# rampasek/GraphGPS

Hardware: NVIDIA H100
Metric: graphs/sec GPSLayer fwd+bwd (higher is better)
Workload: dtype f32

## Files before the change

### graphgps_b200/csrc/attention.cu

```cuda
#include "kernels.cuh"

namespace gps {

namespace {

constexpr int kWarpsPerBlock = 4;

__device__ __forceinline__ int find_graph(const int* __restrict__ gptr, int B, int node) {
  int lo = 0, hi = B;
  while (hi - lo > 1) {
    int mid = (lo + hi) >> 1;
    if (gptr[mid] <= node) lo = mid; else hi = mid;
  }
  return lo;
}

template <int LPR>
__device__ __forceinline__ float group_sum(float v) {
#pragma unroll
  for (int o = LPR / 2; o > 0; o >>= 1) v += __shfl_xor_sync(0xffffffffu, v, o);
  return v;
}

__device__ __forceinline__ int warp_max_i(int v) {
#pragma unroll
  for (int o = 16; o > 0; o >>= 1) v = max(v, __shfl_xor_sync(0xffffffffu, v, o));
  return v;
}

struct DropQuad {
  Philox4 r;
  uint32_t thr;
  float keep_scale;
};
__device__ __forceinline__ void drop_quad_refresh(DropQuad& q, float p, uint64_t seed, uint64_t offset, int head, int i, int jl) {
  q.r = philox4x32(seed, offset + (uint64_t)(GPS_SITE_ATTN_P + head), ((uint64_t)i << 20) | (uint64_t)(jl >> 2));
}
__device__ __forceinline__ float drop_quad_scale(const DropQuad& q, int jl) {
  const int k = jl & 3;
  const uint32_t bits = k == 0 ? q.r.v[0] : k == 1 ? q.r.v[1] : k == 2 ? q.r.v[2] : q.r.v[3];
  return bits >= q.thr ? q.keep_scale : 0.f;
}
__device__ __forceinline__ void drop_quad_init(DropQuad& q, float p) {
  q.thr = (uint32_t)fminf(p * 4294967296.f, 4294967295.f);
  q.keep_scale = 1.f / (1.f - p);
}

template <int VW> struct VecT;
template <> struct VecT<4> { using T = float4; };
template <> struct VecT<1> { using T = float; };

template <int VW> __device__ __forceinline__ typename VecT<VW>::T vld(const float* p);
template <> __device__ __forceinline__ float4 vld<4>(const float* p) { return ld4(p); }
template <> __device__ __forceinline__ float vld<1>(const float* p) { return *p; }
template <int VW> __device__ __forceinline__ typename VecT<VW>::T vzero();
template <> __device__ __forceinline__ float4 vzero<4>() { return f4zero(); }
template <> __device__ __forceinline__ float vzero<1>() { return 0.f; }
__device__ __forceinline__ void vst(float* p, float4 v) { st4(p, v); }
__device__ __forceinline__ void vst(float* p, float v) { *p = v; }
__device__ __forceinline__ float4 vscale(float4 a, float s) { return f4scale(a, s); }
__device__ __forceinline__ float vscale(float a, float s) { return a * s; }
__device__ __forceinline__ float vdot(float4 a, float4 b) { return a.x * b.x + a.y * b.y + a.z * b.z + a.w * b.w; }
__device__ __forceinline__ float vdot(float a, float b) { return a * b; }
__device__ __forceinline__ void vplanes_store(const Planes& p, int64_t r, int64_t c, float4 v) { planes_store4(p, r, c, v); }
__device__ __forceinline__ void vplanes_store(const Planes& p, int64_t r, int64_t c, float v) {
  const __nv_bfloat16 h = __float2bfloat16_rn(v);
  p.hi[r * p.ld + c] = h;
  if (p.lo) p.lo[r * p.ld + c] = __float2bfloat16_rn(v - __bfloat162float(h));
}

template <int CH, int LPR, int VW>
__device__ __forceinline__ void load_slice(typename VecT<VW>::T* dst, const float* row, int sub, int nch, bool ok) {
#pragma unroll
  for (int c = 0; c < CH; ++c) {
    int ch = sub + c * LPR;
    dst[c] = (ok && ch < nch) ? vld<VW>(row + ch * VW) : vzero<VW>();
  }
}
template <int CH, int LPR, int VW>
__device__ __forceinline__ void store_slice(const typename VecT<VW>::T* src, float* row, int sub, int nch) {
#pragma unroll
  for (int c = 0; c < CH; ++c) {
    int ch = sub + c * LPR;
    if (ch < nch) vst(row + ch * VW, src[c]);
  }
}
template <int CH, int LPR, int VW>
__device__ __forceinline__ void store_slice_planes(const typename VecT<VW>::T* src, const Planes& p, int64_t r, int64_t col0,
                                                   int sub, int nch) {
  if (!p.hi) return;
#pragma unroll
  for (int c = 0; c < CH; ++c) {
    int ch = sub + c * LPR;
    if (ch < nch) vplanes_store(p, r, col0 + ch * VW, src[c]);
  }
}
template <int CH, typename V>
__device__ __forceinline__ float dot_slice(const V* a, const V* b) {
  float s = 0.f;
#pragma unroll
  for (int c = 0; c < CH; ++c) s += vdot(a[c], b[c]);
  return s;
}

struct AttnArgs {
  const int* gptr; int B; int N; int H; int hd;
  const float* Q; const float* K; const float* V; int64_t ld;
  float* O; const float* Oc; const float* dO; int64_t ldo;
  float* lse; const float* lsec; float* delta; const float* deltac;
  float* dQ; float* dK; float* dV; int64_t ldg;
  float scale; float p_drop; uint64_t seed, offset;
  const unsigned long long* offset_dev;
  Planes Op, dQp, dKp, dVp;
  int smem_rows;
  const float* bias; int64_t nmax; float* gbias;
};
__device__ __forceinline__ uint64_t eff_offset(const AttnArgs& a) {
  return a.offset + ((a.p_drop > 0.f && a.offset_dev) ? *a.offset_dev : 0ull);
}

struct StagedRows {
  const float* x; int64_t ldx;
  const float* y; int64_t ldy;
};
template <int RPB, int VW>
__device__ __forceinline__ StagedRows stage_rows(const AttnArgs& a, const float* X, int64_t ldX, const float* Y, int64_t ldY,
                                                 int h, float* sm) {
  const int64_t hoff = (int64_t)h * a.hd;
  StagedRows r{X + hoff, ldX, Y + hoff, ldY};
  const int r0 = blockIdx.x * RPB;
  if (a.smem_rows <= 0 || r0 >= a.N) return r;
  const int last = min(r0 + RPB, a.N) - 1;
  const int kmin = a.gptr[find_graph(a.gptr, a.B, r0)];
  const int R = a.gptr[find_graph(a.gptr, a.B, last) + 1] - kmin;
  if (R > a.smem_rows) return r;
  const int pitch = a.hd + 4, nch = VW == 4 ? a.hd >> 2 : a.hd;
  float* sx = sm;
  float* sy = sm + (int64_t)a.smem_rows * pitch;
  for (int idx = threadIdx.x; idx < R * nch; idx += blockDim.x) {
    const int row = idx / nch, c = idx - row * nch;
    vst(sx + row * pitch + c * VW, vld<VW>(X + (int64_t)(kmin + row) * ldX + hoff + c * VW));
    vst(sy + row * pitch + c * VW, vld<VW>(Y + (int64_t)(kmin + row) * ldY + hoff + c * VW));
  }
  __syncthreads();
  r.x = sx - (int64_t)kmin * pitch; r.ldx = pitch;
  r.y = sy - (int64_t)kmin * pitch; r.ldy = pitch;
  return r;
}

template <int CH, int LPR, bool BIAS, int VW>
__global__ void __launch_bounds__(kWarpsPerBlock * 32) k_attn_fwd(AttnArgs a) {
  extern __shared__ float attn_sm[];
  using V = typename VecT<VW>::T;
  constexpr int RPW = 32 / LPR;
  const int warp = threadIdx.x >> 5, lane = threadIdx.x & 31;
  const int sub = lane % LPR, rloc = lane / LPR;
  const int h = blockIdx.y;
  const int i = (blockIdx.x * kWarpsPerBlock + warp) * RPW + rloc;
  const bool row_ok = i < a.N;
  const int nch = a.hd / VW;
  const uint64_t offs = eff_offset(a);
  int gs = 0, n = 0;
  const float* brow = nullptr;
  if (row_ok) {
    int g = find_graph(a.gptr, a.B, i);
    gs = a.gptr[g];
    n = a.gptr[g + 1] - gs;
    if constexpr (BIAS) brow = a.bias + (((int64_t)g * a.H + h) * a.nmax + (i - gs)) * a.nmax;
  }
  const int nloop = warp_max_i(n);
  const int64_t hoff = (int64_t)h * a.hd;
  V q[CH], o[CH];
  load_slice<CH, LPR, VW>(q, a.Q + (int64_t)(row_ok ? i : 0) * a.ld + hoff, sub, nch, row_ok);
#pragma unroll
  for (int c = 0; c < CH; ++c) {
    q[c] = vscale(q[c], a.scale);
    o[c] = vzero<VW>();
  }
  float m = -INFINITY, l = 0.f;
  const bool use_drop = a.p_drop > 0.f;
  DropQuad dq;
  drop_quad_init(dq, a.p_drop);
  const StagedRows kv = stage_rows<RPW * kWarpsPerBlock, VW>(a, a.K, a.ld, a.V, a.ld, h, attn_sm);
  V kc[CH], vc[CH];
  load_slice<CH, LPR, VW>(kc, kv.x + (int64_t)gs * kv.ldx, sub, nch, n > 0);
  load_slice<CH, LPR, VW>(vc, kv.y + (int64_t)gs * kv.ldy, sub, nch, n > 0);
  float bc = 0.f;
  if constexpr (BIAS) bc = n > 0 ? brow[0] : 0.f;
  for (int jl = 0; jl < nloop; ++jl) {
    if (use_drop && (jl & 3) == 0) drop_quad_refresh(dq, a.p_drop, a.seed, offs, h, i, jl);
    const bool valid = jl < n;
    const bool nvalid = jl + 1 < n;
    const int jn = gs + (nvalid ? jl + 1 : 0);
    V kn[CH], vn[CH];
    load_slice<CH, LPR, VW>(kn, kv.x + (int64_t)jn * kv.ldx, sub, nch, nvalid);
    load_slice<CH, LPR, VW>(vn, kv.y + (int64_t)jn * kv.ldy, sub, nch, nvalid);
    float bn = 0.f;
    if constexpr (BIAS) bn = nvalid ? brow[jl + 1] : 0.f;
    float s = group_sum<LPR>(dot_slice<CH>(q, kc));
    if constexpr (BIAS) s += bc;
    s = valid ? s : -INFINITY;
    const float m_new = fmaxf(m, s);
    const float corr = (m_new == -INFINITY) ? 1.f : __expf(m - m_new);
    const float p = valid ? __expf(s - m_new) : 0.f;
    l = l * corr + p;
    const float pd = use_drop ? p * drop_quad_scale(dq, jl) : p;
#pragma unroll
    for (int c = 0; c < CH; ++c) {
      if constexpr (VW == 4) {
        o[c].x = o[c].x * corr + pd * vc[c].x;
        o[c].y = o[c].y * corr + pd * vc[c].y;
        o[c].z = o[c].z * corr + pd * vc[c].z;
        o[c].w = o[c].w * corr + pd * vc[c].w;
      } else {
        o[c] = o[c] * corr + pd * vc[c];
      }
      kc[c] = kn[c];
      vc[c] = vn[c];
    }
    if constexpr (BIAS) bc = bn;
    m = m_new;
  }
  if (row_ok) {
    const float inv = 1.f / l;
#pragma unroll
    for (int c = 0; c < CH; ++c) o[c] = vscale(o[c], inv);
    store_slice<CH, LPR, VW>(o, a.O + (int64_t)i * a.ldo + hoff, sub, nch);
    store_slice_planes<CH, LPR, VW>(o, a.Op, i, hoff, sub, nch);
    if (sub == 0) a.lse[(int64_t)i * a.H + h] = m + __logf(l);
  }
}

template <int VW>
__global__ void k_attn_delta(AttnArgs a) {
  using V = typename VecT<VW>::T;
  const int64_t t = ((int64_t)blockIdx.x * blockDim.x + threadIdx.x) >> 3;
  const int sub = threadIdx.x & 7;
  const bool ok = t < (int64_t)a.N * a.H;
  const int64_t i = ok ? t / a.H : 0;
  const int h = ok ? (int)(t - i * a.H) : 0;
  const V* go = reinterpret_cast<const V*>(a.dO + i * a.ldo + (int64_t)h * a.hd);
  const V* oo = reinterpret_cast<const V*>(a.Oc + i * a.ldo + (int64_t)h * a.hd);
  float acc = 0.f;
  if (ok)
    for (int c = sub; c < a.hd / VW; c += 8) {
      const V x = __ldg(go + c), y = __ldg(oo + c);
      acc += vdot(x, y);
    }
  acc += __shfl_xor_sync(0xffffffffu, acc, 4);
  acc += __shfl_xor_sync(0xffffffffu, acc, 2);
  acc += __shfl_xor_sync(0xffffffffu, acc, 1);
  if (ok && sub == 0) a.delta[t] = acc;
}

template <int CH, int LPR, bool BIAS, int VW>
__device__ __forceinline__ void attn_bwd_q_body(const AttnArgs& a, float* attn_sm) {
  using V = typename VecT<VW>::T;
  constexpr int RPW = 32 / LPR;
  const int warp = threadIdx.x >> 5, lane = threadIdx.x & 31;
  const int sub = lane % LPR, rloc = lane / LPR;
  const int h = blockIdx.y;
  const int i = (blockIdx.x * kWarpsPerBlock + warp) * RPW + rloc;
  const bool row_ok = i < a.N;
  const int nch = a.hd / VW;
  const uint64_t offs = eff_offset(a);
  int gs = 0, n = 0;
  int64_t brow = 0;
  if (row_ok) {
    int g = find_graph(a.gptr, a.B, i);
    gs = a.gptr[g];
    n = a.gptr[g + 1] - gs;
    if constexpr (BIAS) brow = (((int64_t)g * a.H + h) * a.nmax + (i - gs)) * a.nmax;
  }
  const int nloop = warp_max_i(n);
  const int64_t hoff = (int64_t)h * a.hd;
  const int ir = row_ok ? i : 0;
  V q[CH], go[CH], gq[CH];
  load_slice<CH, LPR, VW>(q, a.Q + (int64_t)ir * a.ld + hoff, sub, nch, row_ok);
  load_slice<CH, LPR, VW>(go, a.dO + (int64_t)ir * a.ldo + hoff, sub, nch, row_ok);
  {
    const float dl = row_ok ? a.deltac[(int64_t)i * a.H + h] : 0.f;
#pragma unroll
    for (int c = 0; c < CH; ++c) gq[c] = vzero<VW>();
    const float lse = row_ok ? a.lsec[(int64_t)i * a.H + h] : 0.f;
#pragma unroll
    for (int c = 0; c < CH; ++c) q[c] = vscale(q[c], a.scale);
    const bool use_drop = a.p_drop > 0.f;
    DropQuad dq;
    drop_quad_init(dq, a.p_drop);
    const StagedRows kv = stage_rows<RPW * kWarpsPerBlock, VW>(a, a.K, a.ld, a.V, a.ld, h, attn_sm);
    V kk[CH], vv[CH];
    load_slice<CH, LPR, VW>(kk, kv.x + (int64_t)gs * kv.ldx, sub, nch, n > 0);
    load_slice<CH, LPR, VW>(vv, kv.y + (int64_t)gs * kv.ldy, sub, nch, n > 0);
    float bc = 0.f;
    if constexpr (BIAS) bc = n > 0 ? a.bias[brow] : 0.f;
    for (int jl = 0; jl < nloop; ++jl) {
      if (use_drop && (jl & 3) == 0) drop_quad_refresh(dq, a.p_drop, a.seed, offs, h, i, jl);
      const bool valid = jl < n;
      const bool nvalid = jl + 1 < n;
      const int jn = gs + (nvalid ? jl + 1 : 0);
      V kn[CH], vn[CH];
      load_slice<CH, LPR, VW>(kn, kv.x + (int64_t)jn * kv.ldx, sub, nch, nvalid);
      load_slice<CH, LPR, VW>(vn, kv.y + (int64_t)jn * kv.ldy, sub, nch, nvalid);
      float bn = 0.f;
      if constexpr (BIAS) bn = nvalid ? a.bias[brow + jl + 1] : 0.f;
      float s = dot_slice<CH>(q, kk), dp = dot_slice<CH>(go, vv);
#pragma unroll
      for (int ofs = LPR / 2; ofs > 0; ofs >>= 1) {
        s += __shfl_xor_sync(0xffffffffu, s, ofs);
        dp += __shfl_xor_sync(0xffffffffu, dp, ofs);
      }
      if constexpr (BIAS) s += bc;
      const float p = valid ? __expf(s - lse) : 0.f;
      const float ds = p * (dp * (use_drop ? drop_quad_scale(dq, jl) : 1.f) - dl);
      if constexpr (BIAS) {
        if (a.gbias && valid && sub == 0) a.gbias[brow + jl] = ds;
        bc = bn;
      }
#pragma unroll
      for (int c = 0; c < CH; ++c) {
        if constexpr (VW == 4) {
          gq[c].x += ds * kk[c].x;
          gq[c].y += ds * kk[c].y;
          gq[c].z += ds * kk[c].z;
          gq[c].w += ds * kk[c].w;
        } else {
          gq[c] += ds * kk[c];
        }
        kk[c] = kn[c];
        vv[c] = vn[c];
      }
    }
  }
  if (row_ok) {
#pragma unroll
    for (int c = 0; c < CH; ++c) gq[c] = vscale(gq[c], a.scale);
    store_slice<CH, LPR, VW>(gq, a.dQ + (int64_t)i * a.ldg + hoff, sub, nch);
    store_slice_planes<CH, LPR, VW>(gq, a.dQp, i, hoff, sub, nch);
  }
}

template <int CH, int LPR, bool BIAS, int VW>
__device__ __forceinline__ void attn_bwd_kv_body(const AttnArgs& a, float* attn_sm) {
  using V = typename VecT<VW>::T;
  constexpr int RPW = 32 / LPR;
  const int warp = threadIdx.x >> 5, lane = threadIdx.x & 31;
  const int sub = lane % LPR, rloc = lane / LPR;
  const int h = blockIdx.y;
  const int j = (blockIdx.x * kWarpsPerBlock + warp) * RPW + rloc;
  const bool row_ok = j < a.N;
  const int nch = a.hd / VW;
  const uint64_t offs = eff_offset(a);
  int gs = 0, n = 0;
  const float* bcol = nullptr;
  if (row_ok) {
    int g = find_graph(a.gptr, a.B, j);
    gs = a.gptr[g];
    n = a.gptr[g + 1] - gs;
    if constexpr (BIAS) bcol = a.bias + ((int64_t)g * a.H + h) * a.nmax * a.nmax + (j - gs);
  }
  const int nloop = warp_max_i(n);
  const int jl = j - gs;
  const int64_t hoff = (int64_t)h * a.hd;
  const int jr = row_ok ? j : 0;
  V kk[CH], vv[CH], gk[CH], gv[CH];
  load_slice<CH, LPR, VW>(kk, a.K + (int64_t)jr * a.ld + hoff, sub, nch, row_ok);
  load_slice<CH, LPR, VW>(vv, a.V + (int64_t)jr * a.ld + hoff, sub, nch, row_ok);
#pragma unroll
  for (int c = 0; c < CH; ++c) {
    gk[c] = vzero<VW>();
    gv[c] = vzero<VW>();
  }
  const StagedRows qd = stage_rows<RPW * kWarpsPerBlock, VW>(a, a.Q, a.ld, a.dO, a.ldo, h, attn_sm);
  V q[CH], go[CH];
  load_slice<CH, LPR, VW>(q, qd.x + (int64_t)gs * qd.ldx, sub, nch, n > 0);
  load_slice<CH, LPR, VW>(go, qd.y + (int64_t)gs * qd.ldy, sub, nch, n > 0);
  for (int il = 0; il < nloop; ++il) {
    const bool valid = il < n;
    const int i = gs + (valid ? il : 0);
    const bool nvalid = il + 1 < n;
    const int in_ = gs + (nvalid ? il + 1 : 0);
    V qn[CH], gon[CH];
    load_slice<CH, LPR, VW>(qn, qd.x + (int64_t)in_ * qd.ldx, sub, nch, nvalid);
    load_slice<CH, LPR, VW>(gon, qd.y + (int64_t)in_ * qd.ldy, sub, nch, nvalid);
    float s = dot_slice<CH>(q, kk), dp = dot_slice<CH>(go, vv);
#pragma unroll
    for (int ofs = LPR / 2; ofs > 0; ofs >>= 1) {
      s += __shfl_xor_sync(0xffffffffu, s, ofs);
      dp += __shfl_xor_sync(0xffffffffu, dp, ofs);
    }
    const float lse = valid ? a.lsec[(int64_t)i * a.H + h] : 0.f;
    const float dl = valid ? a.deltac[(int64_t)i * a.H + h] : 0.f;
    float p;
    if constexpr (BIAS) p = valid ? __expf(s * a.scale + bcol[(int64_t)il * a.nmax] - lse) : 0.f;
    else p = valid ? __expf(s * a.scale - lse) : 0.f;
    float dsc = 1.f;
    if (a.p_drop > 0.f) {
      DropQuad dq;
      drop_quad_init(dq, a.p_drop);
      drop_quad_refresh(dq, a.p_drop, a.seed, offs, h, i, jl);
      dsc = drop_quad_scale(dq, jl);
    }
    const float pd = p * dsc;
    const float ds = p * (dp * dsc - dl) * a.scale;
#pragma unroll
    for (int c = 0; c < CH; ++c) {
      if constexpr (VW == 4) {
        gk[c].x += ds * q[c].x; gk[c].y += ds * q[c].y; gk[c].z += ds * q[c].z; gk[c].w += ds * q[c].w;
        gv[c].x += pd * go[c].x; gv[c].y += pd * go[c].y; gv[c].z += pd * go[c].z; gv[c].w += pd * go[c].w;
      } else {
        gk[c] += ds * q[c];
        gv[c] += pd * go[c];
      }
      q[c] = qn[c];
      go[c] = gon[c];
    }
  }
  if (row_ok) {
    store_slice<CH, LPR, VW>(gk, a.dK + (int64_t)j * a.ldg + hoff, sub, nch);
    store_slice<CH, LPR, VW>(gv, a.dV + (int64_t)j * a.ldg + hoff, sub, nch);
    store_slice_planes<CH, LPR, VW>(gk, a.dKp, j, hoff, sub, nch);
    store_slice_planes<CH, LPR, VW>(gv, a.dVp, j, hoff, sub, nch);
  }
}

template <int CH, int LPR, bool BIAS, int VW>
__global__ void __launch_bounds__(kWarpsPerBlock * 32) k_attn_bwd(AttnArgs a) {
  extern __shared__ float attn_sm[];
  if (blockIdx.z == 0) attn_bwd_kv_body<CH, LPR, BIAS, VW>(a, attn_sm);
  else attn_bwd_q_body<CH, LPR, BIAS, VW>(a, attn_sm);
}

enum { KFWD = 0, KBWD = 1 };

constexpr int kStageBytes = 72 * 1024;

static bool attn_vec4(const AttnArgs& a, int which) {
  return a.hd % 4 == 0 && a.ld % 4 == 0 && a.ldo % 4 == 0 && (which == KFWD || a.ldg % 4 == 0);
}

template <int CH, int LPR, bool BIAS, int VW>
static void launch_one(int which, const AttnArgs& a0, cudaStream_t stream) {
  constexpr int RPW = 32 / LPR;
  AttnArgs a = a0;
  static const bool stage_on = [] {
    const char* e = getenv("GPS_B200_ATTN_STAGE");
    return e && e[0] == '1';
  }();
  const int pitch = a.hd + 4;
  a.smem_rows = (stage_on && a.B > 0 && a.N < 64LL * a.B) ? kStageBytes / (2 * pitch * 4) : 0;
  const size_t smem = a.smem_rows > 0 ? (size_t)2 * a.smem_rows * pitch * 4 : 0;
  static bool attr_done[2] = {false, false};
  if (smem > 0 && !attr_done[which]) {
    if (which == KFWD)
      cudaFuncSetAttribute(k_attn_fwd<CH, LPR, BIAS, VW>, cudaFuncAttributeMaxDynamicSharedMemorySize, kStageBytes);
    else cudaFuncSetAttribute(k_attn_bwd<CH, LPR, BIAS, VW>, cudaFuncAttributeMaxDynamicSharedMemorySize, kStageBytes);
    attr_done[which] = true;
  }
  dim3 grid((unsigned)ceil_div(a.N, (int64_t)RPW * kWarpsPerBlock), (unsigned)a.H, which == KFWD ? 1 : 2);
  dim3 block(kWarpsPerBlock * 32);
  if (which == KFWD) k_attn_fwd<CH, LPR, BIAS, VW><<<grid, block, smem, stream>>>(a);
  else k_attn_bwd<CH, LPR, BIAS, VW><<<grid, block, smem, stream>>>(a);
}

static int dispatch(int which, const AttnArgs& a, cudaStream_t stream) {
  GPS_REQUIRE(a.hd > 0 && a.hd <= 192, GPS_ERR_UNSUPPORTED, "attention: head dim %d must be in 1..192", a.hd);
  if (a.N == 0) return GPS_OK;
  const int vw = attn_vec4(a, which) ? 4 : 1;
  const int nch = a.hd / vw;
  int lpr = 1;
  while ((nch + lpr - 1) / lpr > 6) lpr *= 2;
  const int ch = (nch + lpr - 1) / lpr;
#define GPS_ATTN_CASE(VWV, CHV, LPRV)                                  \
  if (vw == VWV && ch == CHV && lpr == LPRV) {                         \
    if (a.bias) launch_one<CHV, LPRV, true, VWV>(which, a, stream);    \
    else launch_one<CHV, LPRV, false, VWV>(which, a, stream);          \
    GPS_LAUNCH_CHECK();                                                \
    return GPS_OK;                                                     \
  }
  GPS_ATTN_CASE(4, 1, 1) GPS_ATTN_CASE(4, 2, 1) GPS_ATTN_CASE(4, 3, 1) GPS_ATTN_CASE(4, 4, 1) GPS_ATTN_CASE(4, 5, 1)
  GPS_ATTN_CASE(4, 6, 1) GPS_ATTN_CASE(4, 4, 2) GPS_ATTN_CASE(4, 5, 2) GPS_ATTN_CASE(4, 6, 2) GPS_ATTN_CASE(4, 4, 4)
  GPS_ATTN_CASE(4, 5, 4) GPS_ATTN_CASE(4, 6, 4) GPS_ATTN_CASE(4, 4, 8) GPS_ATTN_CASE(4, 5, 8) GPS_ATTN_CASE(4, 6, 8)
  GPS_ATTN_CASE(1, 1, 1) GPS_ATTN_CASE(1, 2, 1) GPS_ATTN_CASE(1, 3, 1) GPS_ATTN_CASE(1, 4, 1) GPS_ATTN_CASE(1, 5, 1)
  GPS_ATTN_CASE(1, 6, 1) GPS_ATTN_CASE(1, 4, 2) GPS_ATTN_CASE(1, 5, 2) GPS_ATTN_CASE(1, 6, 2) GPS_ATTN_CASE(1, 4, 4)
  GPS_ATTN_CASE(1, 5, 4) GPS_ATTN_CASE(1, 6, 4) GPS_ATTN_CASE(1, 4, 8) GPS_ATTN_CASE(1, 5, 8) GPS_ATTN_CASE(1, 6, 8)
  GPS_ATTN_CASE(1, 4, 16) GPS_ATTN_CASE(1, 5, 16) GPS_ATTN_CASE(1, 6, 16) GPS_ATTN_CASE(1, 4, 32)
  GPS_ATTN_CASE(1, 5, 32) GPS_ATTN_CASE(1, 6, 32)
#undef GPS_ATTN_CASE
  set_error("attention: no kernel for head dim %d", a.hd);
  return GPS_ERR_UNSUPPORTED;
}

}

int attention_fwd(const GpsGraph& g, int64_t heads, int64_t hd, const float* Q, const float* K, const float* V,
                  int64_t ld, float* O, int64_t ldo, float* lse, float p_drop, uint64_t seed, uint64_t offset,
                  cudaStream_t stream, const unsigned long long* offset_dev, Planes Op, const GpsAttnBias* bias) {
  AttnArgs a{};
  a.offset_dev = offset_dev;
  a.Op = Op;
  if (bias) { a.bias = bias->bias; a.nmax = bias->nmax; }
  a.gptr = g.graph_ptr; a.B = (int)g.B; a.N = (int)g.N; a.H = (int)heads; a.hd = (int)hd;
  a.Q = Q; a.K = K; a.V = V; a.ld = ld; a.O = O; a.ldo = ldo; a.lse = lse;
  a.scale = 1.f / sqrtf((float)hd); a.p_drop = p_drop; a.seed = seed; a.offset = offset;
  return dispatch(KFWD, a, stream);
}

int attention_bwd(const GpsGraph& g, int64_t heads, int64_t hd, const float* Q, const float* K, const float* V,
                  int64_t ld, const float* O, const float* dO, int64_t ldo, const float* lse, float* delta,
                  float* dQ, float* dK, float* dV, int64_t ldg, float p_drop, uint64_t seed, uint64_t offset,
                  cudaStream_t stream, const unsigned long long* offset_dev, Planes dQp, Planes dKp, Planes dVp,
                  const GpsAttnBias* bias) {
  AttnArgs a{};
  a.offset_dev = offset_dev;
  if (bias) { a.bias = bias->bias; a.nmax = bias->nmax; a.gbias = bias->grad_bias; }
  a.dQp = dQp; a.dKp = dKp; a.dVp = dVp;
  a.gptr = g.graph_ptr; a.B = (int)g.B; a.N = (int)g.N; a.H = (int)heads; a.hd = (int)hd;
  a.Q = Q; a.K = K; a.V = V; a.ld = ld; a.Oc = O; a.dO = dO; a.ldo = ldo; a.lsec = lse;
  a.delta = delta; a.deltac = delta; a.dQ = dQ; a.dK = dK; a.dV = dV; a.ldg = ldg;
  a.scale = 1.f / sqrtf((float)hd); a.p_drop = p_drop; a.seed = seed; a.offset = offset;
  if (a.gbias)
    GPS_CUDA(cudaMemsetAsync(a.gbias, 0, (size_t)(g.B * heads * a.nmax * a.nmax) * sizeof(float), stream));
  GPS_REQUIRE(a.hd > 0 && a.hd <= 192, GPS_ERR_UNSUPPORTED, "attention: head dim %d must be in 1..192", a.hd);
  if (a.N == 0) return GPS_OK;
  const int64_t nt = (int64_t)a.N * a.H * 8;
  if (attn_vec4(a, KBWD)) k_attn_delta<4><<<(unsigned)ceil_div(nt, (int64_t)256), 256, 0, stream>>>(a);
  else k_attn_delta<1><<<(unsigned)ceil_div(nt, (int64_t)256), 256, 0, stream>>>(a);
  GPS_LAUNCH_CHECK();
  return dispatch(KBWD, a, stream);
}

}
```

### graphgps_b200/csrc/layer.cu

```cuda
#include <stdarg.h>
#include <string.h>

#include <algorithm>
#include <atomic>

#include "layer_ops.cuh"

namespace gps {

int perf_supported(int64_t dim_head, int64_t features);
int64_t perf_mp();
int perf_index_range(int64_t N, int64_t H);
int perf_prep(const float* P, int64_t m, float* Pn, const GpsGraph& g, int64_t H, int* nmax, float* gmax, int* argk,
              cudaStream_t st);
int perf_features_fwd(float* fq, float* fk, const float* Q, const float* K, const GpsGraph& g, int64_t H, int64_t m,
                      float* gmax, int* argq, int* argk, cudaStream_t st);
int perf_linattn_fwd(const GpsGraph& g, int64_t H, int64_t m, const int* nmax, const float* qf, const float* kf,
                     const float* V, const float* gmax, float* O, cudaStream_t st);
int perf_linattn_bwd(const GpsGraph& g, int64_t H, int64_t m, const int* nmax, const float* qf, const float* kf,
                     const float* V, const float* gmax, const float* gO, float* g_qf, float* g_kf, float* gV,
                     float* ggmax, cudaStream_t st);
int perf_features_bwd(float* g_fq, float* g_fk, const float* fq, const float* fk, const float* Q, const float* K,
                      float* gQ, float* gK, const GpsGraph& g, int64_t H, int64_t m, const int* argq, const int* argk,
                      const float* ggmax, float* gmrow, bool pairwise, cudaStream_t st);
// ... 934 lines not shown
    GPS_TRY(gemm(g3, sg));
    float* dst = P.hA;
    Planes dstp;
    const float* r2 = nullptr;
    if (P.nonorm) {
      dst = P.s; dstp = P.s_p;
      if (two_branches) {
        r2 = P.xloc;
        GPS_TRY(sd->order(st, sg));
      }
    }
    GPS_TRY(layernorm_fwd(P.bb_z2, N, d, B.ln2.weight, B.ln2.bias, B.ln_eps, stat + 2 * N, stat + 3 * N, dst, dstp, a->x,
                          r2, P.drop(GPS_SITE_ATTN_OUT), stats(BN_A), sg));
  }

  if (two_branches) GPS_TRY(sd->order(sd->s3, st));

  if (!P.nonorm) {
    const float* first = P.loc ? P.xloc : P.hA;
    BnView bf = P.loc ? bn_view(P, BN_L, a->norm1_local, N) : bn_view(P, BN_A, a->norm1_attn, N);
    const float* second = (P.loc && P.glob) ? P.hA : nullptr;
    BnView bs = bn_view(P, BN_A, a->norm1_attn, N);
    GPS_TRY(bn_combine(first, bf, second, bs, P.s, N, d, st, P.s_p));
  }

  {
    GemmParams g = linear_fwd(P, N, 2 * d, d, {P.s, d, P.s_p}, {a->ff1.weight, d, P.ff1_p}, P.hid, 2 * d, a->ff1.bias);
    g.act = act; g.C_pre = P.hid_pre; g.ldpre = (int)(2 * d); g.Cp = P.hid_p;
    set_dropout(g, P.drop(GPS_SITE_FF1));
    GPS_TRY(gemm(g, st));
    GemmParams g2 = linear_fwd(P, N, d, 2 * d, {P.hid, 2 * d, P.hid_p}, {a->ff2.weight, 2 * d, P.ff2_p}, P.t, d,
                               a->ff2.bias);
    g2.R1 = P.s; g2.ldr1 = (int)d; g2.stats = stats(BN_2);
    set_dropout(g2, P.drop(GPS_SITE_FF2));
    if (P.nonorm) {
      g2.C = a->x_out;
      g2.Cp = out_planes(a->x_planes_out);
    }
    GPS_TRY(gemm(g2, st));
    if (!P.nonorm)
      GPS_TRY(bn_combine(P.t, bn_view(P, BN_2, a->norm2, N), nullptr, BnView(), a->x_out, N, d, st,
                         out_planes(a->x_planes_out)));
  }
  return GPS_OK;
}

static int layer_backward(const GpsLayerArgs* a, cudaStream_t st) {
  Plan P;
  const GpsGat& gat = a->gat;
  const GpsGenConv& gen = a->genconv;
  const GpsPna& pna = a->pna;
  GPS_TRY(make_plan(a, &P, true));
  GPS_REQUIRE(a->saved && a->workspace, GPS_ERR_ARG, "saved/workspace buffers are required");
  GPS_REQUIRE(a->workspace_bytes >= P.bwd_bytes, GPS_ERR_ARG, "workspace too small (%lld < %lld)",
              (long long)a->workspace_bytes, (long long)P.bwd_bytes);
  GPS_TRY(check_params(a, P));
  GPS_REQUIRE(a->grad_x_out && a->grad_x, GPS_ERR_ARG, "grad_x_out / grad_x are required");
  GPS_REQUIRE(!P.gat || P.E == 0 || a->grad_edge_attr, GPS_ERR_ARG, "grad_edge_attr is required for GAT");
  GPS_REQUIRE(!P.gen || P.E == 0 || a->grad_edge_attr, GPS_ERR_ARG, "grad_edge_attr is required for GENConv");
  GPS_REQUIRE(!P.pna || P.E == 0 || a->grad_edge_attr, GPS_ERR_ARG, "grad_edge_attr is required for PNA");
  const int64_t N = P.N, E = P.E, d = P.d;
  const int act = a->act;
  DropCfg nodrop;
  auto sums = [&](int which) { return P.bsums + (int64_t)which * 2 * d; };
  GPS_CUDA(cudaMemsetAsync(P.bsums, 0, (size_t)P.nbn * 2 * d * sizeof(double), st));
  if (P.gen) GPS_CUDA(cudaMemsetAsync(P.gen_bsums, 0, (size_t)2 * 2 * d * sizeof(double), st));
  Side* sd;
  GPS_TRY(side_stream(&sd));
  cudaStream_t s2 = sd->s;
  auto wfork = [&](cudaStream_t from) -> int { return sd->order(from, s2); };
  const bool two_branches = P.loc && P.glob;
  cudaStream_t sa = two_branches ? sd->s3 : st;
  cudaStream_t se = sd->s4;
  const int opt = opt_flags();
  auto record_ev = [&](void* ev, cudaStream_t s) -> int {
    if (!ev) return GPS_OK;
    cudaStreamCaptureStatus cs = cudaStreamCaptureStatusNone;
    GPS_CUDA(cudaStreamIsCapturing(s, &cs));
    GPS_CUDA(cudaEventRecordWithFlags((cudaEvent_t)ev, s, cs == cudaStreamCaptureStatusActive ? cudaEventRecordExternal
                                                                                               : cudaEventRecordDefault));
    return GPS_OK;
  };
  auto early_done = [&]() -> int { return record_ev(a->ev_grads_early, s2); };
  auto mid_done = [&]() -> int { return record_ev(a->ev_grads_mid, s2); };
  const bool gx_splitk = P.Wy >= 1024 && N > 0;
  if (P.Wy) {
    GPS_TRY(wfork(st));
    GPS_CUDA(cudaMemsetAsync(P.gWcat, 0, (size_t)(P.Wy * d + P.Wy) * sizeof(float), s2));
  }
  if (gx_splitk) GPS_CUDA(cudaMemsetAsync(a->grad_x, 0, (size_t)(N * d) * sizeof(float), st));

  if (P.gated) {
    GPS_TRY(sd->order(st, se));
    BnView ve = bn_view(P, BN_E, a->bn_edge_e);
    if (a->grad_edge_out && E > 0) {
      GPS_TRY(bn_bwd_reduce(a->grad_edge_out, d, P.ehat, d, E, d, ve, act, P.drop(GPS_SITE_GCN_E), sums(BN_E), se));
      GPS_TRY(bn_bwd_apply(a->grad_edge_out, d, P.ehat, d, E, d, ve, act, P.drop(GPS_SITE_GCN_E), sums(BN_E), P.g_e, d,
                           a->bn_edge_e.grad_weight, a->bn_edge_e.grad_bias, se, P.grads_accumulate));
    } else {
      if (E > 0) GPS_CUDA(cudaMemsetAsync(P.g_e, 0, (size_t)(E * d) * sizeof(float), se));
      if (a->bn_edge_e.grad_weight && !P.grads_prezeroed)
        GPS_CUDA(cudaMemsetAsync(a->bn_edge_e.grad_weight, 0, d * sizeof(float), se));
      if (a->bn_edge_e.grad_bias && !P.grads_prezeroed)
        GPS_CUDA(cudaMemsetAsync(a->bn_edge_e.grad_bias, 0, d * sizeof(float), se));
    }
  }

  const float* g_t = P.nonorm ? a->grad_x_out : P.g_t;
  if (!P.nonorm) {
    BnView v2 = bn_view(P, BN_2, a->norm2);
    GPS_TRY(bn_bwd_reduce(a->grad_x_out, d, P.t, d, N, d, v2, -1, nodrop, sums(BN_2), st));
    GPS_TRY(bn_bwd_apply(a->grad_x_out, d, P.t, d, N, d, v2, -1, nodrop, sums(BN_2), P.g_t, d, a->norm2.grad_weight,
                         a->norm2.grad_bias, st, P.grads_accumulate, P.gt_p));
  } else if (!(P.dropout.p > 0.f) && P.gt_p.hi && N > 0) {
    ToPlanesItem it{g_t, d, (int)N, (int)d, P.gt_p};
    GPS_TRY(to_planes(&it, 1, st));
  }
  const float* g_xloc = P.nonorm ? P.g_s : P.g_xloc;
  const Planes g_xloc_p = P.nonorm ? P.gs_p : P.gl1_p;
  const float* g_hA = P.nonorm ? P.g_s : P.g_hA;
  const Planes g_hA_p = P.nonorm ? P.gs_p : P.ghA_p;

  bool fused_la = false;
  {
    Operand g_ff2;
    GPS_TRY(dropmul(P, {g_t, d, P.gt_p}, P.g_tmp, P.gtmp_p, GPS_SITE_FF2, st, &g_ff2));
    GemmParams g = linear_dgrad(P, N, 2 * d, d, g_ff2, {a->ff2.weight, 2 * d, P.ff2_p}, P.g_hid, 2 * d);
    set_act_mask(g, act, P.hid, P.hid_pre, 2 * d);
    set_dropout(g, P.drop(GPS_SITE_FF1));
    g.Cp = P.ghid_p;
    GPS_TRY(gemm(g, st));
    const Operand g_hid{P.g_hid, 2 * d, P.ghid_p};
    GPS_TRY(wfork(st));
    GPS_TRY(linear_wgrad(P, g_ff2, {P.hid, 2 * d, P.hid_p}, N, d, 2 * d, a->ff2.grad_weight, a->ff2.grad_bias, s2));
    GPS_TRY(linear_wgrad(P, g_hid, {P.s, d, P.s_p}, N, 2 * d, d, a->ff1.grad_weight, a->ff1.grad_bias, s2));
    GemmParams g2 = linear_dgrad(P, N, d, 2 * d, g_hid, {a->ff1.weight, d, P.ff1_p}, P.g_s, d);
    g2.R1 = g_t; g2.ldr1 = (int)d;
    g2.Cp = P.gs_p;
    fused_la = (opt & 64) && !P.nonorm && P.use_planes && g2.Ap.hi && g2.Bp.hi && N > 0 && P.train;
    if (fused_la) {
      if (P.loc) {
        BnView v = bn_view(P, BN_L, a->norm1_local);
        g2.bnred[0].z = P.xloc; g2.bnred[0].ldz = (int)d; g2.bnred[0].mean = v.mean; g2.bnred[0].invstd = v.invstd;
        g2.bnred[0].sums = sums(BN_L);
      }
      if (P.glob) {
        BnView v = bn_view(P, BN_A, a->norm1_attn);
        g2.bnred[1].z = P.hA; g2.bnred[1].ldz = (int)d; g2.bnred[1].mean = v.mean; g2.bnred[1].invstd = v.invstd;
        g2.bnred[1].sums = sums(BN_A);
      }
    }
    GPS_TRY(gemm(g2, st));
  }

  bool chain_x = false;
  if (P.loc && !P.nonorm) {
    BnView v = bn_view(P, BN_L, a->norm1_local);
    if (!fused_la) GPS_TRY(bn_bwd_reduce(P.g_s, d, P.xloc, d, N, d, v, -1, nodrop, sums(BN_L), st));
    chain_x = P.gated && N > 0 && (opt & 32) && P.train;
    if (chain_x)
      GPS_TRY(bn_bwd_apply_chain(P.g_s, d, P.xloc, d, N, d, v, sums(BN_L), P.g_xloc, d, a->norm1_local.grad_weight,
                                 a->norm1_local.grad_bias, P.grads_accumulate, P.gl1_p, P.xt, d,
                                 bn_view(P, BN_X, a->bn_node_x), act, P.drop(GPS_SITE_GCN_X), sums(BN_X), st));
    else
      GPS_TRY(bn_bwd_apply(P.g_s, d, P.xloc, d, N, d, v, -1, nodrop, sums(BN_L), P.g_xloc, d,
                           a->norm1_local.grad_weight, a->norm1_local.grad_bias, st, P.grads_accumulate, P.gl1_p));
  }
  if (!P.attn && !P.perf && !P.bb) {
    GPS_TRY(wfork(st));
    GPS_TRY(early_done());
  }
  if (two_branches) GPS_TRY(sd->order(st, sa));
  if (P.attn) {
    if (!P.nonorm) {
      BnView v = bn_view(P, BN_A, a->norm1_attn);
      if (!fused_la) GPS_TRY(bn_bwd_reduce(P.g_s, d, P.hA, d, N, d, v, -1, nodrop, sums(BN_A), sa));
      GPS_TRY(bn_bwd_apply(P.g_s, d, P.hA, d, N, d, v, -1, nodrop, sums(BN_A), P.g_hA, d, a->norm1_attn.grad_weight,
                           a->norm1_attn.grad_bias, sa, P.grads_accumulate, P.ghA_p));
    }
    Operand g_ao;
    GPS_TRY(dropmul(P, {g_hA, d, g_hA_p}, P.g_tmp2, P.gtmp2_p, GPS_SITE_ATTN_OUT, sa, &g_ao));
    GPS_TRY(gemm(linear_dgrad(P, N, d, d, g_ao, {a->attn_out.weight, d, P.out_p}, P.g_O, d), sa));
    GPS_TRY(wfork(sa));
    GPS_TRY(linear_wgrad(P, g_ao, {P.O, d, P.O_p}, N, d, d, a->attn_out.grad_weight, a->attn_out.grad_bias, s2));
    GPS_TRY(early_done());
    const float* Q = P.Y1 + P.qkv_off;
    float* gQ = P.gY1 + P.qkv_off;
    GPS_TRY(attention_bwd(a->graph, P.H, P.hd, Q, Q + d, Q + 2 * d, P.Wy, P.O, P.g_O, d, P.lse, P.delta, gQ, gQ + d,
                          gQ + 2 * d, P.Wy, P.pa, a->seed, a->offset, sa, (const unsigned long long*)a->offset_dev,
                          P.gY1_p.cols(P.qkv_off), P.gY1_p.cols(P.qkv_off + d), P.gY1_p.cols(P.qkv_off + 2 * d), P.bias));
  }

  if (P.perf) {
    const int64_t inner = P.inner, NH = N * P.H, dh = a->perf_dim_head;
    if (!P.nonorm) {
      BnView v = bn_view(P, BN_A, a->norm1_attn);
      if (!fused_la) GPS_TRY(bn_bwd_reduce(P.g_s, d, P.hA, d, N, d, v, -1, nodrop, sums(BN_A), sa));
      GPS_TRY(bn_bwd_apply(P.g_s, d, P.hA, d, N, d, v, -1, nodrop, sums(BN_A), P.g_hA, d, a->norm1_attn.grad_weight,
                           a->norm1_attn.grad_bias, sa, P.grads_accumulate));
    }
    Operand g_ao;
    GPS_TRY(dropmul(P, {g_hA, d}, P.g_tmp2, Planes(), GPS_SITE_ATTN_OUT, sa, &g_ao, P.pa, GPS_SITE_PERF_OUT));
    GPS_TRY(gemm(linear_dgrad(P, N, inner, d, g_ao, {a->attn_out.weight, inner}, P.g_O, inner), sa));
    GPS_TRY(wfork(sa));
    GPS_TRY(linear_wgrad(P, g_ao, {P.O, inner}, N, d, inner, a->attn_out.grad_weight, a->attn_out.grad_bias, s2));
    GPS_TRY(early_done());
    if (P.perf_pairwise)
      GPS_TRY(perf_quad_bwd(a->graph, P.H, P.m, P.pnmax, P.pfq, P.pfk, P.pV, P.pgmax, P.O, P.pden, P.g_O, P.g_pden,
                            P.g_pfq, P.g_pfk, P.g_pV, P.g_pgrow, sa));
    else
      GPS_TRY(perf_linattn_bwd(a->graph, P.H, P.m, P.pnmax, P.pfq, P.pfk, P.pV, P.pgmax, P.g_O, P.g_pfq, P.g_pfk, P.g_pV,
                               P.g_pgmax, sa));
    GPS_TRY(perf_features_bwd(P.g_pfq, P.g_pfk, P.pfq, P.pfk, P.pQ, P.pK, P.g_pQ, P.g_pK, a->graph, P.H, P.m, P.pargq,
                              P.pargk, P.g_pgmax, P.g_pgrow, P.perf_pairwise, sa));
    float* gdd[2] = {P.g_pfq, P.g_pfk};
    float* gqk[2] = {P.g_pQ, P.g_pK};
    for (int i = 0; i < 2; ++i) {
      GemmParams h = linear_dgrad(P, NH, dh, P.mp, {gdd[i], P.mp}, {P.pPn, dh}, gqk[i], dh);
      h.R1 = gqk[i]; h.ldr1 = (int)dh;
      GPS_TRY(gemm(h, sa));
    }
    const GpsLinear* lin[3] = {&a->perf_q, &a->perf_k, &a->perf_v};
    const float* gsrc[3] = {P.g_pQ, P.g_pK, P.g_pV};
    GPS_TRY(wfork(sa));
    for (int i = 0; i < 3; ++i) {
      GPS_TRY(linear_wgrad(P, {gsrc[i], inner}, {a->x, d}, N, inner, d, lin[i]->grad_weight, nullptr, s2));
      GemmParams h = linear_dgrad(P, N, d, inner, {gsrc[i], inner}, {lin[i]->weight, d}, P.g_xp, d);
      h.R1 = i == 0 ? g_hA : P.g_xp; h.ldr1 = (int)d;
      GPS_TRY(gemm(h, sa));
    }
  }

  if (P.bb) {
    const GpsBigBird& B = a->bigbird;
    if (!P.nonorm) {
      BnView v = bn_view(P, BN_A, a->norm1_attn);
      if (!fused_la) GPS_TRY(bn_bwd_reduce(P.g_s, d, P.hA, d, N, d, v, -1, nodrop, sums(BN_A), sa));
      GPS_TRY(bn_bwd_apply(P.g_s, d, P.hA, d, N, d, v, -1, nodrop, sums(BN_A), P.g_hA, d, a->norm1_attn.grad_weight,
                           a->norm1_attn.grad_bias, sa, P.grads_accumulate));
    }
    GPS_TRY(wfork(sa));
    GPS_TRY(early_done());
    const float* stat = P.bb_stat;
    GPS_TRY(layernorm_bwd(g_hA, P.drop(GPS_SITE_ATTN_OUT), P.bb_z2, N, d, B.ln2.weight, stat + 2 * N, stat + 3 * N,
                          P.bb_god, P.bb_god_p, P.drop(GPS_SITE_BB_OUTPUT), P.bb_dz2, nullptr, P.bb_part,
                          B.ln2.grad_weight, B.ln2.grad_bias, P.grads_accumulate, sa));
    const bool relu = B.hidden_act == GPS_BIGBIRD_RELU;
    const Operand g_od{P.bb_god, d, P.bb_god_p}, g_u{P.bb_gu, d, P.bb_gu_p};
    GemmParams g = linear_dgrad(P, N, d, d, g_od, {B.output.weight, d, P.bb_out_p}, P.bb_gu, d);
    if (relu) {
      set_act_mask(g, GPS_ACT_RELU, P.bb_u, nullptr, d);
      g.Cp = P.bb_gu_p;
    }
    GPS_TRY(gemm(g, sa));
    if (!relu) GPS_TRY(sigmoid_bwd(P.bb_gu, P.bb_u, N, d, P.bb_gu_p, sa));
    GPS_TRY(wfork(sa));
    GPS_TRY(linear_wgrad(P, g_od, {P.bb_u, d, P.bb_u_p}, N, d, d, B.output.grad_weight, B.output.grad_bias, s2));
    GPS_TRY(linear_wgrad(P, g_u, {P.bb_a, d, P.bb_a_p}, N, d, d, B.intermediate.grad_weight, B.intermediate.grad_bias,
                         s2));
    GemmParams g2 = linear_dgrad(P, N, d, d, g_u, {B.intermediate.weight, d, P.bb_in_p}, P.bb_ga, d);
    g2.R1 = P.bb_dz2; g2.ldr1 = (int)d;
    GPS_TRY(gemm(g2, sa));
    GPS_TRY(layernorm_bwd(P.bb_ga, nodrop, P.bb_z1, N, d, B.ln1.weight, stat, stat + N, P.bb_gso, P.bb_gso_p,
                          P.drop(GPS_SITE_BB_SELF_OUT), P.bb_gx, g_hA, P.bb_part, B.ln1.grad_weight, B.ln1.grad_bias,
                          P.grads_accumulate, sa));
    const Operand g_so{P.bb_gso, d, P.bb_gso_p};
    GPS_TRY(gemm(linear_dgrad(P, N, d, d, g_so, {B.self_out.weight, d, P.bb_so_p}, P.g_O, d), sa));
    GPS_TRY(wfork(sa));
    GPS_TRY(linear_wgrad(P, g_so, {P.O, d, P.O_p}, N, d, d, B.self_out.grad_weight, B.self_out.grad_bias, s2));
    if (!P.loc) GPS_TRY(mid_done());
    const float* Q = P.Y1 + P.qkv_off;
    float* gQ = P.gY1 + P.qkv_off;
    GPS_TRY(bb_attn_bwd(a->graph, P.H, P.hd, B, Q, Q + d, Q + 2 * d, P.Wy, P.O, P.g_O, d, P.lse, P.delta, gQ, gQ + d,
                        gQ + 2 * d, P.Wy, sa));
    if (P.gY1_p.hi && N > 0) {
      ToPlanesItem it{gQ, P.Wy, (int)N, (int)(3 * d), P.gY1_p.cols(P.qkv_off)};
      GPS_TRY(to_planes(&it, 1, sa));
    }
  }

  const float* g_x_local = nullptr;
  if (P.gated) {
    BnView vx = bn_view(P, BN_X, a->bn_node_x);
    if (!chain_x)
      GPS_TRY(bn_bwd_reduce(g_xloc, d, P.xt, d, N, d, vx, act, P.drop(GPS_SITE_GCN_X), sums(BN_X), st));
    GPS_TRY(bn_bwd_apply(g_xloc, d, P.xt, d, N, d, vx, act, P.drop(GPS_SITE_GCN_X), sums(BN_X), P.gY1, P.Wy,
                         a->bn_node_x.grad_weight, a->bn_node_x.grad_bias, st, P.grads_accumulate, P.gY1_p));
    GPS_TRY(sd->order(se, st));
    GPS_TRY(gatedgcn_bwd_dst(a->graph, d, P.gY1, P.Wy, P.ehat, P.Y1 + d, P.Wy, P.g_e, P.g_num, P.gY1 + 2 * d, st, P.ge_p,
                             P.gY1_p.cols(2 * d), P.pe_rho, P.g_den));
    if (P.eslap) {
      GPS_TRY(sd->order(st, se));
      GPS_TRY(eslap_bwd(a->graph, a->pe, a->pe_dim, d, act, P.g_num, P.g_den, P.Y1 + d, P.Wy, P.ehat, P.pe_r, P.pe_rho,
                        a->pe_mlp0.weight, a->pe_mlp0.bias, a->pe_mlp1.weight, P.pe_gz, P.pe_gr, P.pe_part, a->grad_pe,
                        a->pe_mlp0.grad_weight, a->pe_mlp0.grad_bias, a->pe_mlp1.grad_weight, a->pe_mlp1.grad_bias,
                        P.grads_accumulate, se));
    }
    GPS_TRY(gatedgcn_bwd_src(a->graph, d, P.g_e, P.ehat, P.g_num, P.gY1 + 3 * d, P.gY1 + d, P.Wy, st, P.gY1_p.cols(3 * d),
                             P.gY1_p.cols(d), P.pe_rho));
    const Operand g_e{P.g_e, d, P.ge_p};
    GPS_TRY(wfork(st));
    GPS_TRY(linear_wgrad(P, g_e, {a->edge_attr, d, P.e_p}, E, d, d, a->gcn_C.grad_weight, a->gcn_C.grad_bias, s2));
    if (P.eslap) GPS_TRY(sd->order(se, s2));
    GPS_TRY(mid_done());
    if (a->grad_edge_attr && E > 0) {
      GemmParams g = linear_dgrad(P, E, d, d, g_e, {a->gcn_C.weight, d, P.C_p}, a->grad_edge_attr, d);
      g.R1 = a->grad_edge_out; g.ldr1 = (int)d;
      GPS_TRY(gemm(g, st));
    }
    g_x_local = g_xloc;
  } else if (P.gine) {
    Operand g_l1;
    GPS_TRY(dropmul(P, {g_xloc, d, g_xloc_p}, P.g_tmp3, P.gtmp3_p, GPS_SITE_LOCAL, st, &g_l1));
    GemmParams g = linear_dgrad(P, N, d, d, g_l1, {a->gine_lin1.weight, d, P.g1_p}, P.g_h1, d);
    set_act_mask(g, act, P.h1, P.h1_pre, d);
    g.Cp = P.gh1_p;
    GPS_TRY(gemm(g, st));
    const Operand g_h1{P.g_h1, d, P.gh1_p};
    GPS_TRY(wfork(st));
    GPS_TRY(linear_wgrad(P, g_l1, {P.h1, d, P.h1_p}, N, d, d, a->gine_lin1.grad_weight, a->gine_lin1.grad_bias, s2));
    GPS_TRY(linear_wgrad(P, g_h1, {P.agg, d, P.agg_p}, N, d, d, a->gine_lin0.grad_weight, a->gine_lin0.grad_bias, s2));
    GPS_TRY(mid_done());
    GPS_TRY(gemm(linear_dgrad(P, N, d, d, g_h1, {a->gine_lin0.weight, d, P.g0_p}, P.g_agg, d), st));
    GPS_REQUIRE(a->grad_edge_attr || E == 0, GPS_ERR_ARG, "grad_edge_attr is required for GINE");
    GPS_TRY(gine_bwd_dst(a->graph, d, a->x, a->edge_attr, P.g_agg, a->grad_edge_attr, st));
// ... 575 lines not shown
```

Measured before the change: 340,100.

## Remove opt-in smem K/V staging and fork attention stream earlier in backward

Deletes the env-gated shared-memory staging of K/V (and Q/dO) rows from the attention kernels, so they always read directly from global memory with zero dynamic smem. In the layer backward, the attention-branch stream now orders on the main stream right after the FF dgrad GEMM, before the local-branch batchnorm backward runs. A work fork is also added on that path, so the attention backward can overlap with the local BN backward. The staging path was off by default, so the kernel edit is mostly a cleanup. The stream reorder is the real scheduling change and needs correct dependencies, since the attention BN backward reads the same g_s gradient.

```diff
diff --git a/graphgps_b200/csrc/attention.cu b/graphgps_b200/csrc/attention.cu
--- a/graphgps_b200/csrc/attention.cu
+++ b/graphgps_b200/csrc/attention.cu
@@ -112,45 +112,14 @@
   float scale; float p_drop; uint64_t seed, offset;
   const unsigned long long* offset_dev;
   Planes Op, dQp, dKp, dVp;
-  int smem_rows;
   const float* bias; int64_t nmax; float* gbias;
 };
 __device__ __forceinline__ uint64_t eff_offset(const AttnArgs& a) {
   return a.offset + ((a.p_drop > 0.f && a.offset_dev) ? *a.offset_dev : 0ull);
 }
 
-struct StagedRows {
-  const float* x; int64_t ldx;
-  const float* y; int64_t ldy;
-};
-template <int RPB, int VW>
-__device__ __forceinline__ StagedRows stage_rows(const AttnArgs& a, const float* X, int64_t ldX, const float* Y, int64_t ldY,
-                                                 int h, float* sm) {
-  const int64_t hoff = (int64_t)h * a.hd;
-  StagedRows r{X + hoff, ldX, Y + hoff, ldY};
-  const int r0 = blockIdx.x * RPB;
-  if (a.smem_rows <= 0 || r0 >= a.N) return r;
-  const int last = min(r0 + RPB, a.N) - 1;
-  const int kmin = a.gptr[find_graph(a.gptr, a.B, r0)];
-  const int R = a.gptr[find_graph(a.gptr, a.B, last) + 1] - kmin;
-  if (R > a.smem_rows) return r;
-  const int pitch = a.hd + 4, nch = VW == 4 ? a.hd >> 2 : a.hd;
-  float* sx = sm;
-  float* sy = sm + (int64_t)a.smem_rows * pitch;
-  for (int idx = threadIdx.x; idx < R * nch; idx += blockDim.x) {
-    const int row = idx / nch, c = idx - row * nch;
-    vst(sx + row * pitch + c * VW, vld<VW>(X + (int64_t)(kmin + row) * ldX + hoff + c * VW));
-    vst(sy + row * pitch + c * VW, vld<VW>(Y + (int64_t)(kmin + row) * ldY + hoff + c * VW));
-  }
-  __syncthreads();
-  r.x = sx - (int64_t)kmin * pitch; r.ldx = pitch;
-  r.y = sy - (int64_t)kmin * pitch; r.ldy = pitch;
-  return r;
-}
-
 template <int CH, int LPR, bool BIAS, int VW>
 __global__ void __launch_bounds__(kWarpsPerBlock * 32) k_attn_fwd(AttnArgs a) {
-  extern __shared__ float attn_sm[];
   using V = typename VecT<VW>::T;
   constexpr int RPW = 32 / LPR;
   const int warp = threadIdx.x >> 5, lane = threadIdx.x & 31;
@@ -181,10 +150,11 @@
   const bool use_drop = a.p_drop > 0.f;
   DropQuad dq;
   drop_quad_init(dq, a.p_drop);
-  const StagedRows kv = stage_rows<RPW * kWarpsPerBlock, VW>(a, a.K, a.ld, a.V, a.ld, h, attn_sm);
+  const float* Kh = a.K + hoff;
+  const float* Vh = a.V + hoff;
   V kc[CH], vc[CH];
-  load_slice<CH, LPR, VW>(kc, kv.x + (int64_t)gs * kv.ldx, sub, nch, n > 0);
-  load_slice<CH, LPR, VW>(vc, kv.y + (int64_t)gs * kv.ldy, sub, nch, n > 0);
+  load_slice<CH, LPR, VW>(kc, Kh + (int64_t)gs * a.ld, sub, nch, n > 0);
+  load_slice<CH, LPR, VW>(vc, Vh + (int64_t)gs * a.ld, sub, nch, n > 0);
   float bc = 0.f;
   if constexpr (BIAS) bc = n > 0 ? brow[0] : 0.f;
   for (int jl = 0; jl < nloop; ++jl) {
@@ -193,8 +163,8 @@
     const bool nvalid = jl + 1 < n;
     const int jn = gs + (nvalid ? jl + 1 : 0);
     V kn[CH], vn[CH];
-    load_slice<CH, LPR, VW>(kn, kv.x + (int64_t)jn * kv.ldx, sub, nch, nvalid);
-    load_slice<CH, LPR, VW>(vn, kv.y + (int64_t)jn * kv.ldy, sub, nch, nvalid);
+    load_slice<CH, LPR, VW>(kn, Kh + (int64_t)jn * a.ld, sub, nch, nvalid);
+    load_slice<CH, LPR, VW>(vn, Vh + (int64_t)jn * a.ld, sub, nch, nvalid);
     float bn = 0.f;
     if constexpr (BIAS) bn = nvalid ? brow[jl + 1] : 0.f;
     float s = group_sum<LPR>(dot_slice<CH>(q, kc));
@@ -254,7 +224,7 @@
 }
 
 template <int CH, int LPR, bool BIAS, int VW>
-__device__ __forceinline__ void attn_bwd_q_body(const AttnArgs& a, float* attn_sm) {
+__device__ __forceinline__ void attn_bwd_q_body(const AttnArgs& a) {
   using V = typename VecT<VW>::T;
   constexpr int RPW = 32 / LPR;
   const int warp = threadIdx.x >> 5, lane = threadIdx.x & 31;
@@ -288,10 +258,11 @@
     const bool use_drop = a.p_drop > 0.f;
     DropQuad dq;
     drop_quad_init(dq, a.p_drop);
-    const StagedRows kv = stage_rows<RPW * kWarpsPerBlock, VW>(a, a.K, a.ld, a.V, a.ld, h, attn_sm);
+    const float* Kh = a.K + hoff;
+    const float* Vh = a.V + hoff;
     V kk[CH], vv[CH];
-    load_slice<CH, LPR, VW>(kk, kv.x + (int64_t)gs * kv.ldx, sub, nch, n > 0);
-    load_slice<CH, LPR, VW>(vv, kv.y + (int64_t)gs * kv.ldy, sub, nch, n > 0);
+    load_slice<CH, LPR, VW>(kk, Kh + (int64_t)gs * a.ld, sub, nch, n > 0);
+    load_slice<CH, LPR, VW>(vv, Vh + (int64_t)gs * a.ld, sub, nch, n > 0);
     float bc = 0.f;
     if constexpr (BIAS) bc = n > 0 ? a.bias[brow] : 0.f;
     for (int jl = 0; jl < nloop; ++jl) {
@@ -300,8 +271,8 @@
       const bool nvalid = jl + 1 < n;
       const int jn = gs + (nvalid ? jl + 1 : 0);
       V kn[CH], vn[CH];
-      load_slice<CH, LPR, VW>(kn, kv.x + (int64_t)jn * kv.ldx, sub, nch, nvalid);
-      load_slice<CH, LPR, VW>(vn, kv.y + (int64_t)jn * kv.ldy, sub, nch, nvalid);
+      load_slice<CH, LPR, VW>(kn, Kh + (int64_t)jn * a.ld, sub, nch, nvalid);
+      load_slice<CH, LPR, VW>(vn, Vh + (int64_t)jn * a.ld, sub, nch, nvalid);
       float bn = 0.f;
       if constexpr (BIAS) bn = nvalid ? a.bias[brow + jl + 1] : 0.f;
       float s = dot_slice<CH>(q, kk), dp = dot_slice<CH>(go, vv);
@@ -341,7 +312,7 @@
 }
 
 template <int CH, int LPR, bool BIAS, int VW>
-__device__ __forceinline__ void attn_bwd_kv_body(const AttnArgs& a, float* attn_sm) {
+__device__ __forceinline__ void attn_bwd_kv_body(const AttnArgs& a) {
   using V = typename VecT<VW>::T;
   constexpr int RPW = 32 / LPR;
   const int warp = threadIdx.x >> 5, lane = threadIdx.x & 31;
@@ -371,18 +342,19 @@
     gk[c] = vzero<VW>();
     gv[c] = vzero<VW>();
   }
-  const StagedRows qd = stage_rows<RPW * kWarpsPerBlock, VW>(a, a.Q, a.ld, a.dO, a.ldo, h, attn_sm);
+  const float* Qh = a.Q + hoff;
+  const float* Gh = a.dO + hoff;
   V q[CH], go[CH];
-  load_slice<CH, LPR, VW>(q, qd.x + (int64_t)gs * qd.ldx, sub, nch, n > 0);
-  load_slice<CH, LPR, VW>(go, qd.y + (int64_t)gs * qd.ldy, sub, nch, n > 0);
+  load_slice<CH, LPR, VW>(q, Qh + (int64_t)gs * a.ld, sub, nch, n > 0);
+  load_slice<CH, LPR, VW>(go, Gh + (int64_t)gs * a.ldo, sub, nch, n > 0);
   for (int il = 0; il < nloop; ++il) {
     const bool valid = il < n;
     const int i = gs + (valid ? il : 0);
     const bool nvalid = il + 1 < n;
     const int in_ = gs + (nvalid ? il + 1 : 0);
     V qn[CH], gon[CH];
-    load_slice<CH, LPR, VW>(qn, qd.x + (int64_t)in_ * qd.ldx, sub, nch, nvalid);
-    load_slice<CH, LPR, VW>(gon, qd.y + (int64_t)in_ * qd.ldy, sub, nch, nvalid);
+    load_slice<CH, LPR, VW>(qn, Qh + (int64_t)in_ * a.ld, sub, nch, nvalid);
+    load_slice<CH, LPR, VW>(gon, Gh + (int64_t)in_ * a.ldo, sub, nch, nvalid);
     float s = dot_slice<CH>(q, kk), dp = dot_slice<CH>(go, vv);
 #pragma unroll
     for (int ofs = LPR / 2; ofs > 0; ofs >>= 1) {
@@ -426,41 +398,23 @@
 
 template <int CH, int LPR, bool BIAS, int VW>
 __global__ void __launch_bounds__(kWarpsPerBlock * 32) k_attn_bwd(AttnArgs a) {
-  extern __shared__ float attn_sm[];
-  if (blockIdx.z == 0) attn_bwd_kv_body<CH, LPR, BIAS, VW>(a, attn_sm);
-  else attn_bwd_q_body<CH, LPR, BIAS, VW>(a, attn_sm);
+  if (blockIdx.z == 0) attn_bwd_kv_body<CH, LPR, BIAS, VW>(a);
+  else attn_bwd_q_body<CH, LPR, BIAS, VW>(a);
 }
 
 enum { KFWD = 0, KBWD = 1 };
-
-constexpr int kStageBytes = 72 * 1024;
 
 static bool attn_vec4(const AttnArgs& a, int which) {
   return a.hd % 4 == 0 && a.ld % 4 == 0 && a.ldo % 4 == 0 && (which == KFWD || a.ldg % 4 == 0);
 }
 
 template <int CH, int LPR, bool BIAS, int VW>
-static void launch_one(int which, const AttnArgs& a0, cudaStream_t stream) {
+static void launch_one(int which, const AttnArgs& a, cudaStream_t stream) {
   constexpr int RPW = 32 / LPR;
-  AttnArgs a = a0;
-  static const bool stage_on = [] {
-    const char* e = getenv("GPS_B200_ATTN_STAGE");
-    return e && e[0] == '1';
-  }();
-  const int pitch = a.hd + 4;
-  a.smem_rows = (stage_on && a.B > 0 && a.N < 64LL * a.B) ? kStageBytes / (2 * pitch * 4) : 0;
-  const size_t smem = a.smem_rows > 0 ? (size_t)2 * a.smem_rows * pitch * 4 : 0;
-  static bool attr_done[2] = {false, false};
-  if (smem > 0 && !attr_done[which]) {
-    if (which == KFWD)
-      cudaFuncSetAttribute(k_attn_fwd<CH, LPR, BIAS, VW>, cudaFuncAttributeMaxDynamicSharedMemorySize, kStageBytes);
-    else cudaFuncSetAttribute(k_attn_bwd<CH, LPR, BIAS, VW>, cudaFuncAttributeMaxDynamicSharedMemorySize, kStageBytes);
-    attr_done[which] = true;
-  }
   dim3 grid((unsigned)ceil_div(a.N, (int64_t)RPW * kWarpsPerBlock), (unsigned)a.H, which == KFWD ? 1 : 2);
   dim3 block(kWarpsPerBlock * 32);
-  if (which == KFWD) k_attn_fwd<CH, LPR, BIAS, VW><<<grid, block, smem, stream>>>(a);
-  else k_attn_bwd<CH, LPR, BIAS, VW><<<grid, block, smem, stream>>>(a);
+  if (which == KFWD) k_attn_fwd<CH, LPR, BIAS, VW><<<grid, block, 0, stream>>>(a);
+  else k_attn_bwd<CH, LPR, BIAS, VW><<<grid, block, 0, stream>>>(a);
 }
 
 static int dispatch(int which, const AttnArgs& a, cudaStream_t stream) {
diff --git a/graphgps_b200/csrc/layer.cu b/graphgps_b200/csrc/layer.cu
--- a/graphgps_b200/csrc/layer.cu
+++ b/graphgps_b200/csrc/layer.cu
@@ -1110,6 +1110,7 @@
     }
     GPS_TRY(gemm(g2, st));
   }
+  if (two_branches) GPS_TRY(sd->order(st, sa));
 
   bool chain_x = false;
   if (P.loc && !P.nonorm) {
@@ -1127,8 +1128,9 @@
   if (!P.attn && !P.perf && !P.bb) {
     GPS_TRY(wfork(st));
     GPS_TRY(early_done());
-  }
-  if (two_branches) GPS_TRY(sd->order(st, sa));
+  } else if (two_branches && !P.nonorm) {
+    GPS_TRY(wfork(st));
+  }
   if (P.attn) {
     if (!P.nonorm) {
       BnView v = bn_view(P, BN_A, a->norm1_attn);
```

Result: no change. 342,800, median of 6 (+0.8%).
